# JediZ/PDE-based-image-processing

Hardware: AMD Instinct MI355X
Metric: SOR iterations/sec (3840x2160 flow) (higher is better)
Workload: dtype f32

## Files before the change

include/pdeip.h:

```cpp
#ifndef PDEIP_H
#define PDEIP_H

#ifdef __cplusplus
extern "C" {
#endif

#define PDEIP_OK 0
#define PDEIP_ERR_ARG 1
#define PDEIP_ERR_SOLVER 2
#define PDEIP_ERR_UNSUPPORTED 3
#define PDEIP_ERR_DEVICE 4
#define PDEIP_ERR_NOMEM 5

#define PDEIP_MODE_EXACT_ORDER 0
#define PDEIP_MODE_RED_BLACK 1
#define PDEIP_MODE_LINE_SCAN 2

#define PDEIP_SOLVER_SOR 1
#define PDEIP_SOLVER_ALR 2

const char *pdeip_version(void);
const char *pdeip_last_error(void);
int pdeip_set_mode(int mode);
int pdeip_get_mode(void);
int pdeip_set_device(int device_id);
int pdeip_set_devices(int n, const int *ids);
int pdeip_get_devices(int *ids, int capacity);
int pdeip_release(void);
int pdeip_last_launch_count(void);
int pdeip_debug_last_directions(int *out, int cap);
int pdeip_workspace_generation(void);
int pdeip_persist_error(void);
int pdeip_debug_raise_abort(void);
int pdeip_debug_persist_order(int B, int T, int affine, int *table);
enum { PDEIP_PLAN_ELIN4 = 0, PDEIP_PLAN_LLIN4, PDEIP_PLAN_DISP4, PDEIP_PLAN_PDE4, PDEIP_PLAN_PDE8, PDEIP_PLAN_DISPSYM4 };
enum { PDEIP_PLAN_INFO = 11, PDEIP_PLAN_RECORD = 9 };
int pdeip_debug_plan_sor(int model, int nrows, int ncols, int nframes, int iter, int mode, int aligned16, int has_dst, int num_cus,
                         int rb2_slots, int rbp_slots, int *info, int *records, int capacity);
enum { PDEIP_PLAN_ALR_ELIN4 = 0, PDEIP_PLAN_ALR_LLIN4, PDEIP_PLAN_ALR_LLIN8, PDEIP_PLAN_ALR_DISP4, PDEIP_PLAN_ALR_PDE4, PDEIP_PLAN_ALR_PDE8 };
enum { PDEIP_PLAN_ALR_INFO = 12, PDEIP_PLAN_ALR_PASS = 20 };
int pdeip_debug_plan_alr(int model, int nrows, int ncols, int nframes, int iter, int mode, int *info, int *passes);
int pdeip_debug_rcp_check(unsigned long long *counts);
int pdeip_profile_enable(int on);
int pdeip_profile_read(double *elapsed_ms, int *sweep_launches);


int pdeip_oflow_sor_elin4(const float *U, const float *V, const float *M, const float *Cu,
                          const float *Cv, const float *Du, const float *Dv, const float *wW,
                          const float *wN, const float *wE, const float *wS, int nrows, int ncols,
                          int nframes_coef, int iter, float omega, int solver, float *U_out,
                          float *V_out, float *RU, float *RV);

int pdeip_oflow_sor_llin4(const float *U, const float *V, const float *dU, const float *dV,
                          const float *M, const float *Cu, const float *Cv, const float *Du,
                          const float *Dv, const float *wW, const float *wN, const float *wE,
                          const float *wS, int nrows, int ncols, int nframes_coef, int iter,
                          float omega, int solver, float *dU_out, float *dV_out, float *RU,
                          float *RV);

int pdeip_oflow_sor_llin8(const float *U, const float *V, const float *dU, const float *dV,
                          const float *M, const float *Cu, const float *Cv, const float *Du,
                          const float *Dv, const float *wW, const float *wNW, const float *wN,
                          const float *wNE, const float *wE, const float *wSE, const float *wS,
                          const float *wSW, int nrows, int ncols, int nframes_coef, int iter,
                          float omega, int solver, float *dU_out, float *dV_out, float *RU,
                          float *RV);

int pdeip_oflow_lhs_elin4(const float *U, const float *V, const float *M, const float *Du,
                          const float *Dv, const float *wW, const float *wN, const float *wE,
                          const float *wS, int nrows, int ncols, int nframes_coef, float *AU,
                          float *AV);
// ... 421 lines not shown
```

pde-based-image-processing_amd/capi.py:

```python
import ctypes
import os

HERE = os.path.dirname(os.path.abspath(__file__))
LIB_PATH = os.environ.get("PDEIP_LIB") or os.path.join(HERE, "libpdeip.so")

PDEIP_OK = 0
PDEIP_ERR_ARG = 1
PDEIP_ERR_SOLVER = 2
PDEIP_ERR_UNSUPPORTED = 3
PDEIP_ERR_DEVICE = 4
PDEIP_ERR_NOMEM = 5
MODE_EXACT_ORDER = 0
MODE_RED_BLACK = 1
SEG_SURFACE, SEG_GREEDY, SEG_INVERSE = 0, 1, 2
MODE_LINE_SCAN = 2

_P = ctypes.c_void_p
_I = ctypes.c_int
_F = ctypes.c_float


class PdeipError(RuntimeError):

    def __init__(self, code, message):
# ... 139 lines not shown
    "pdeip_nan_resize_dev": [_P, _P, _I, _I, _I, _I, _I, ctypes.c_double, _P],
    "pdeip_inpaint_meanfill_dev": [_P, _P, _I, _I, _I, _P],
    "pdeip_tv4_inpaint_assemble_dev": [_P, _P, _P, _P, _I, ctypes.c_double, _I, _I, _I, _F] + [_P] * 6,
    "pdeip_inpaint_merge_dev": [_P, _P, _P, _I, _I, _I, _P, _P],
    "pdeip_tv_inpaint4_dev": [_P, _P, _I, _I, _I, _P, _I, _P, _P, _P],
    "pdeip_tv_inpaint4": [_P, _I, _I, _I, _P, _I, _P, _P, _P],
    "pdeip_flow_splat_dev": [_P, _P, _P, _P, _P, _I, _I, _I, ctypes.c_double, _P, _P, _P],
    "pdeip_interp_blend_dev": [_P, _P, _P, _I, _P, _P, _P, _P, _I, _I, ctypes.c_double, _P, _P],
    "pdeip_flow_interpolate_dev": [_P, _P, _P, _I, _P, _P, _P, _P, _I, _I, ctypes.c_double, _P, _P, _P, _P, _P],
    "pdeip_flow_interpolate": [_P, _P, _I, _P, _P, _P, _P, _I, _I, ctypes.c_double, _P, _P, _P, _P, _P],
    "pdeip_gauss_taps": [ctypes.c_double, _P, _I, ctypes.POINTER(ctypes.c_int)],
    "pdeip_gauss": [_P, _I, _I, _I, ctypes.c_double, _P],
    "pdeip_gauss_dev": [_P, _P, _I, _I, _I, ctypes.c_double, _P],
    "pdeip_structure_tensor_dev": [_P, _P, _I, _I, _I, ctypes.c_double, ctypes.c_double, _P],
    "pdeip_st_weights_dev": [_P, _P, _I, _I, _P, ctypes.c_double, _P, _P],
    "pdeip_st_weights_padded_dev": [_P, _P, _I, _I, _P, ctypes.c_double, _P, _P],
    "pdeip_st_pad_dev": [_P, _P, _I, _I, _I, _P, _P],
    "pdeip_st_crop_dev": [_P, _P, _I, _I, _I, _P],
    "pdeip_diffusion8": [_P, _I, _I, _I, _P, _P],
    "pdeip_diffusion8_dev": [_P, _P, _I, _I, _I, _P, _P],
    "pdeip_set_mode": [_I],
    "pdeip_get_mode": [],
    "pdeip_set_device": [_I],
    "pdeip_set_devices": [_I, ctypes.POINTER(ctypes.c_int)],
    "pdeip_get_devices": [ctypes.POINTER(ctypes.c_int), _I],
    "pdeip_release": [],
    "pdeip_last_launch_count": [],
    "pdeip_debug_last_directions": [ctypes.POINTER(ctypes.c_int), _I],
    "pdeip_workspace_generation": [],
    "pdeip_persist_error": [],
    "pdeip_debug_persist_order": [_I, _I, _I, ctypes.POINTER(ctypes.c_int)],
    "pdeip_debug_raise_abort": [],
    "pdeip_debug_plan_sor": [_I] * 11 + [ctypes.POINTER(ctypes.c_int), ctypes.POINTER(ctypes.c_int), _I],
    "pdeip_debug_plan_alr": [_I] * 6 + [ctypes.POINTER(ctypes.c_int), ctypes.POINTER(ctypes.c_int)],
    "pdeip_debug_rcp_check": [ctypes.POINTER(ctypes.c_ulonglong)],
    "pdeip_profile_enable": [_I],
    "pdeip_profile_read": [ctypes.POINTER(ctypes.c_double), ctypes.POINTER(ctypes.c_int)],
}
STRING_FUNCS = ("pdeip_version", "pdeip_last_error")

_lib = None


def load():
    global _lib
    if _lib is not None:
        return _lib
    if not os.path.exists(LIB_PATH):
        raise PdeipError(PDEIP_ERR_DEVICE,
                         "libpdeip.so is not built (%s). Run `python __graft_entry__.py build`; "
                         "there is no CPU fallback." % LIB_PATH)
    try:
        import torch
    except ImportError:
        pass
    try:
        lib = ctypes.CDLL(LIB_PATH)
    except OSError as exc:
        raise PdeipError(PDEIP_ERR_DEVICE, "cannot load %s: %s" % (LIB_PATH, exc)) from exc
    for name, argtypes in SIGNATURES.items():
        fn = getattr(lib, name)
        fn.argtypes = argtypes
        fn.restype = ctypes.c_int
    for name in STRING_FUNCS:
        fn = getattr(lib, name)
        fn.argtypes = []
# ... 58 lines not shown
```

pde-based-image-processing_amd/csrc/pdeip_sor5.hip:

```cpp
#include "pdeip_ctx.hpp"

#include "pdeip_models.hpp"
#include "pdeip_pointwise.hpp"
#include "pdeip_sor_exact.hpp"
#include "pdeip_walk_host.hpp"
#include "pdeip_persist_host.hpp"
#include "pdeip_sor_rb.hpp"
#include "pdeip_sor_rbp.hpp"
#include "pdeip_sor_small.hpp"
#include "pdeip_sor_plan.hpp"

using namespace pdeip;

namespace {

constexpr int PS = RBP_SWEEPS;

template <class Mdl> SorTraits sor_traits()
{
    using PL = RbpLayout<Mdl, PS>;
    return SorTraits{Mdl::NIT, Mdl::NCF, false, 1, RB_OWN_ROWS, PL::FITS, PL::NW, RBP_OWN_ROWS, PL::nsteps(0), &SmallLayout<Mdl>::plan, &walk_width<Mdl>};
}

template <class Mdl> auto rb_kernel(bool vec, bool first, bool two)
// ... 100 lines not shown
    RC(for_each_launch(plan, [&](const SorLaunch &l) {
        bind_buffers<Mdl>(P, buf, l);
        const bool gated = sp.nslabs > 1 && l.src == l.dst;
        if (gated) d->persist_used = true;
        hipLaunchKernelGGL(k_sor_small<Mdl>, dim3((unsigned)sp.nslabs, (unsigned)c.nframes), dim3(SL::THREADS), sp.lds, c.s, P, c.nrows, c.ncols, l.sweeps,
                           c.omega, c.col0, c.n, sp.W, gated ? counter : nullptr, abort_word);
        tls.last_launches++;
        return PDEIP_OK;
    }));
    timer.stop(plan.nlaunch);
    HIPCHK(hipGetLastError());
    return PDEIP_OK;
}

#ifndef PDEIP_TIMER_MARKERS
#define PDEIP_TIMER_MARKERS 0
#endif

template <class Mdl> int run_chain(const SweepCall<Mdl> &c, const SorPlan &plan, float *(&buf)[3][Mdl::NIT])
{
    using PL = RbpLayout<Mdl, PS>;
    SweepPlanes<Mdl> P = c.P;
    hipStream_t s = c.s;
    SweepTimer timer(s, PDEIP_TIMER_MARKERS ? 0 : plan.nlaunch);
    int done = 0;
    DeviceState *d = cur_dev();
    RC(for_each_launch(plan, [&](const SorLaunch &l) {
        bind_buffers<Mdl>(P, buf, l);
        hipEvent_t const e0 = timer.start_for(l.index), e1 = timer.stop_for(l.index);
        const int mirror = l.kind == K_RBP ? resolve_mirror(plan.mirror_mode, d->rbp_next_mirror) : 0;
        if (l.kind == K_RBP) {
            RC(ensure_lds(reinterpret_cast<const void *>(rbp_kernel<Mdl>(l.first)), PL::LDS_BYTES));
            const bool keep = l.first && done + PS < c.iter;
            launch_timed(rbp_kernel<Mdl>(l.first), dim3((unsigned)l.gridx, (unsigned)c.nframes), dim3(PL::THREADS), PL::LDS_BYTES, s, e0, e1, P, keep ? c.aux0 : nullptr,
                         keep ? c.aux1 : nullptr, c.nrows, c.ncols, l.tj, l.tiles, l.units, c.omega, c.col0, c.n, mirror);
        } else {
            launch_timed(rb_kernel<Mdl>(plan.vec, l.first, l.sweeps == 2), dim3((unsigned)l.gridx, (unsigned)c.nframes), dim3(64 * RB_WAVES_PER_BLOCK), 0, s, e0, e1, P,
                         l.first ? c.aux0 : nullptr, l.first ? c.aux1 : nullptr, c.nrows, c.ncols, l.tj, l.tiles, l.units, c.omega, c.col0, c.n);
        }
        if (l.first) {
            P.cf[Mdl::D0] = c.aux0;
            P.cf[Mdl::D1] = c.aux1;
        }
        done += l.sweeps;
        tls.last_launches++;
        tls.last_directions.push_back(mirror);
        return PDEIP_OK;
    }));
    timer.stop(plan.nlaunch);
    if (plan.copy_back)
        for (int f = 0; f < Mdl::NIT; f++) RC(copy_d2d(s, buf[BUF_CALLER][f], buf[BUF_SCRATCH][f], c.n * c.nframes));
    HIPCHK(hipGetLastError());
    return PDEIP_OK;
}

template <class Mdl>
int run_sweeps(hipStream_t s, SweepPlanes<Mdl> P, int nrows, int ncols, int nframes, int iter,
               float omega, int mode, int col0, float *const *dst = nullptr)
{
    constexpr int NIT = Mdl::NIT;
    const size_t n = (size_t)nrows * ncols;
    tls.last_launches = 0;
    tls.last_directions.clear();
    bool same = dst != nullptr, aligned = true;
    for (int f = 0; f < NIT; f++) {
        same = same && dst[f] == P.it_out[f];
        aligned = aligned && aligned16(P.it_out[f]) && (!dst || aligned16(dst[f]));
    }
// ... 23 lines not shown
}

extern "C" int pdeip_debug_plan_sor(int model, int nrows, int ncols, int nframes, int iter, int mode, int aligned16, int has_dst, int num_cus,
                                    int rb2_slots, int rbp_slots, int *info, int *records, int capacity)
{
    const char *who = "pdeip_debug_plan_sor";
    RC(check_dims(who, nrows, ncols, nframes));
    RC(check_mode(who, mode));
    if (info == nullptr || (records == nullptr && capacity > 0)) return set_err(PDEIP_ERR_ARG, "%s: null pointer", who);
    const SorShape sh{nrows, ncols, nframes, iter, mode, aligned16 != 0, has_dst != 0, 0, 0};
    const SorDevice dev{num_cus, rb2_slots, rbp_slots};
    SorPlan p;
    switch (model) {
    case PDEIP_PLAN_ELIN4: p = plan_for<ModelElin4>(sh, dev); break;
    case PDEIP_PLAN_LLIN4: p = plan_for<ModelLlin4>(sh, dev); break;
    case PDEIP_PLAN_DISP4: p = plan_for<ModelDisp4>(sh, dev); break;
    case PDEIP_PLAN_PDE4: p = plan_for<ModelPde4>(sh, dev); break;
    case PDEIP_PLAN_PDE8: p = plan_sor_pde8(sh, dev); break;
    case PDEIP_PLAN_DISPSYM4: p = plan_for<ModelDispSym4>(sh, dev); break;
    default: return set_err(PDEIP_ERR_ARG, "%s: unknown model %d", who, model);
    }
    const int head[PDEIP_PLAN_INFO] = {p.family, p.form, p.copy_back, p.copy_in, p.persist_setup, p.A, p.B, p.NC, p.W, p.last_m, 0};
    memcpy(info, head, sizeof head);
    for (int run = 0; run < (model == PDEIP_PLAN_DISPSYM4 ? 2 : 1); run++)
        (void)for_each_launch(p, [&](const SorLaunch &l) {
            const int rec[PDEIP_PLAN_RECORD] = {l.kind, l.sweeps, l.first, l.tj, l.tiles, l.units, l.gridx, l.src, l.dst};
            if (info[10] < capacity) memcpy(records + (size_t)PDEIP_PLAN_RECORD * info[10], rec, sizeof rec);
            info[10]++;
            return PDEIP_OK;
        });
    return PDEIP_OK;
}

extern "C" int pdeip_debug_persist_order(int B, int T, int affine, int *table)
{
    if (B < 1 || T < 1 || table == nullptr) return set_err(PDEIP_ERR_ARG, "pdeip_debug_persist_order: bad arguments");
    RC(use_device());
    int *dev = nullptr;
    const size_t n = PERSIST_TABLE_HDR + (size_t)B * T;
    HIPCHK(hipMalloc(&dev, n * sizeof(int)));
    hipLaunchKernelGGL(k_persist_order, dim3((unsigned)((B * T + 255) / 256)), dim3(256), 0, nullptr, dev, B, T, affine ? 1 : 0);
    const hipError_t e = hipMemcpy(table, dev, n * sizeof(int), hipMemcpyDeviceToHost);
    (void)hipFree(dev);
    if (e != hipSuccess) return set_err(PDEIP_ERR_DEVICE, "pdeip_debug_persist_order: %s", hipGetErrorString(e));
    return PDEIP_OK;
}

namespace {
__global__ void k_rcp_check(unsigned long long *counts)
{
    const unsigned long long stride = (unsigned long long)gridDim.x * blockDim.x;
    unsigned long long n = 0, bad = 0;
    for (unsigned long long i = (unsigned long long)blockIdx.x * blockDim.x + threadIdx.x; i < (1ull << 32); i += stride) {
        const unsigned bits = (unsigned)i;
        const float d = __uint_as_float(bits);
        bool in_range = true;
        RcpRange{in_range}(d);
        if (in_range != (((bits >> 23) & 0xff) >= 1 && ((bits >> 23) & 0xff) <= 252)) bad++;
        if (!in_range) continue;
        n++;
        if (__float_as_uint(RcpFast()(d)) != __float_as_uint(RcpIeee()(d))) bad++;
    }
    atomicAdd(counts + 0, n);
    atomicAdd(counts + 1, bad);
}
}
// ... 180 lines not shown
```

pde-based-image-processing_amd/csrc/pdeip_sor_plan.hpp:

```cpp
#pragma once
#include "pdeip_ctx.hpp"
#include "pdeip_sor_exact.hpp"
#include "pdeip_sor_rb.hpp"
#include "pdeip_sor_small.hpp"

namespace pdeip {

enum { SOR_NONE = 0, SOR_EXACT, SOR_SMALL, SOR_RB, SOR_RBP, SOR_PDE8 };
enum { FORM_NONE = 0, FORM_PERSIST, FORM_WALK, FORM_FRONT };
enum { K_RBP = 1, K_RB2, K_RB1, K_SMALL, K_P8C2, K_P8C1, K_PACK, K_PERSIST, K_WALK, K_DERIVE, K_FRONT, K_BORDERS };
enum { BUF_CALLER = 0, BUF_SCRATCH, BUF_DST };
constexpr int RBP_SWEEPS = 4;
constexpr int MIRROR_ALTERNATE = 3;

struct SorTraits {
    int nit, ncf;
    bool pde8;
    int ex_skew;
    int rb2_own;
    bool rbp_fits;
    int rbp_nw, rbp_own, rbp_tail;
    SmallPlan (*small)(int, int, int, int);
    int (*walk_width)(int, int, int, int);
};
struct SorShape {
    int nrows, ncols, nframes, iter, mode;
    bool aligned16, has_dst;
    size_t packed_frame_bytes;
    int persist_chunks;
};
struct SorKnobs {
    bool persist = true, walk = false, small = true, fuse = true, pipe = true;
    int small_q = 1, rb_tj = 0, rbp_tj = 0, serpentine = 0;
};
struct SorDevice { int cus, rb2_slots, rbp_slots; };
enum { FACT_CUS, FACT_RB2, FACT_RBP };

struct SorLaunch { int kind, sweeps, first, tj, tiles, units, gridx, src, dst, count, index; };
struct SorPlan {
    int family = SOR_NONE, form = FORM_NONE;
    int A = 0, B = 0, NC = 0, W = 0, last_m = 0;
    int nsteps = 0, nlaunch = 0;
    SorLaunch step[4] = {};
    bool has_dst = false, vec = false;
    int mirror_mode = 0;
    bool copy_in = false;
    bool copy_back = false;
    bool persist_setup = false;
    SmallPlan small;
    void add(int kind, int count, int sweeps = 0, int tj = 0, int tiles = 0, int units = 0, int gridx = 0)
    {
        if (count <= 0) return;
        step[nsteps++] = SorLaunch{kind, sweeps, 0, tj, tiles, units, gridx, 0, 0, count, 0};
        nlaunch += count;
    }
};

enum { KNOBS_EXACT, KNOBS_SMALL, KNOBS_CHAIN, KNOBS_PIPE };
inline void read_sor_knobs(SorKnobs &k, int set, bool pde8 = false)
{
    if (set == KNOBS_EXACT) {
        k.persist = env_int(pde8 ? "PDEIP_PDE8_PERSIST" : "PDEIP_EXACT_PERSIST", 1) != 0;
        k.walk = !pde8 && k.persist && env_int("PDEIP_EXACT_WALK", 0) != 0;
    } else if (set == KNOBS_SMALL) {
        k.small = env_int("PDEIP_RB_SMALL", 1) != 0;
        if (k.small) k.small_q = env_int("PDEIP_SMALL_Q", 1);
    } else if (set == KNOBS_CHAIN) {
        static const bool fuse_enabled = env_int("PDEIP_RB_FUSE", 1) != 0;
        k.fuse = fuse_enabled;
        k.rb_tj = g.rb_tj > 0 ? g.rb_tj : env_int("PDEIP_RB_TJ", 0);
        k.pipe = !pde8 && env_int("PDEIP_RB_PIPE", 1) != 0;
    } else {
        k.rbp_tj = env_int("PDEIP_RBP_TJ", 0);
        const char *serp = getenv("PDEIP_RBP_SERPENTINE");
        const bool set = serp && *serp;
        const int v = set ? atoi(serp) : 0;
        k.serpentine = !set ? -1 : (v < 0 || v > MIRROR_ALTERNATE ? 0 : v);
    }
}

inline bool persist_fits(int strips, int iter, size_t plane_bytes, int ncols)
{
    return strips <= 0xffff && iter <= 0x7fff && plane_bytes < 0xffff0000ull && ncols <= 65535;
}

inline int pick_rb_tj(int forced) { return forced > 0 ? (forced < 2 ? 2 : forced) : 12; }

inline int pick_rb2_tj(int slots, int tiles, int ncols, int nframes)
{
    int best = 12;
    long best_cost = -1;
    for (int tj = 2; tj <= 64; tj++) {
        const long units = (long)tiles * ((ncols + tj - 1) / tj) * nframes;
        const long cost = ((units + slots - 1) / slots) * (tj + 6);
        if (best_cost < 0 || cost <= best_cost) {
            best_cost = cost;
            best = tj;
        }
    }
    return best;
}

inline int pick_rbp_tj(int slots, int tiles, int ncols, int nframes, int tail)
{
    int best = 64;
    long best_cost = -1;
    for (int tj = 8; tj <= 1024; tj++) {
        const long units = (long)tiles * ((ncols + tj - 1) / tj) * nframes;
        const long cost = ((units + slots - 1) / slots) * (tj + tail);
        if (best_cost < 0 || cost < best_cost) {
// ... 46 lines not shown
    p.add(K_SMALL, sh.iter / per_launch, per_launch, sp.W, 1, sp.nslabs, sp.nslabs);
    p.add(K_SMALL, sh.iter % per_launch ? 1 : 0, sh.iter % per_launch, sp.W, 1, sp.nslabs, sp.nslabs);
    return true;
}

template <class Ask> inline void plan_chain(SorPlan &p, const SorTraits &t, const SorShape &sh, SorKnobs &k, const SorDevice &dev, Ask &&ask)
{
    const size_t n = (size_t)sh.nrows * sh.ncols;
    const auto strips = [&](int tj) { return (sh.ncols + tj - 1) / tj; };
    p.vec = sh.nrows % 4 == 0 && sh.aligned16;
    const bool pipe = k.pipe && k.fuse && p.vec && t.rbp_fits && (t.rbp_nw == 2 || n >= (size_t)1 << 21);
    const int n4 = pipe ? sh.iter / RBP_SWEEPS : 0, rest = sh.iter - RBP_SWEEPS * n4, n2 = k.fuse ? rest / 2 : 0, n1 = rest - 2 * n2;
    p.family = t.pde8 ? SOR_PDE8 : (n4 > 0 ? SOR_RBP : SOR_RB);
    if (n4 > 0) {
        read_sor_knobs(k, KNOBS_PIPE);
        const int tiles = (sh.nrows + t.rbp_own - 1) / t.rbp_own;
        const int tj = k.rbp_tj > 0 ? (k.rbp_tj < 2 ? 2 : k.rbp_tj)
                                    : pick_rbp_tj(dev.rbp_slots > 0 ? dev.rbp_slots : ask(FACT_RBP), tiles, sh.ncols, sh.nframes, t.rbp_tail);
        p.add(K_RBP, n4, RBP_SWEEPS, tj, tiles, tiles * strips(tj), tiles * strips(tj));
    }
    const int tj1 = pick_rb_tj(k.rb_tj), tiles1 = rb_row_tiles(sh.nrows, RB_OWN_ROWS), tiles2 = rb_row_tiles(sh.nrows, t.rb2_own);
    const int tj2 = (k.rb_tj > 0 || n2 == 0) ? tj1 : pick_rb2_tj(dev.rb2_slots > 0 ? dev.rb2_slots : ask(FACT_RB2), tiles2, sh.ncols, sh.nframes);
    const auto blocks = [](int units) { return (units + RB_WAVES_PER_BLOCK - 1) / RB_WAVES_PER_BLOCK; };
    p.add(t.pde8 ? K_P8C2 : K_RB2, n2, 2, tj2, tiles2, tiles2 * strips(tj2), blocks(tiles2 * strips(tj2)));
    p.add(t.pde8 ? K_P8C1 : K_RB1, n1, 1, tj1, tiles1, tiles1 * strips(tj1), blocks(tiles1 * strips(tj1)));
    p.copy_back = !sh.has_dst && (p.nlaunch & 1);
}

inline int default_mirror(const SorShape &sh)
{
    return (size_t)13 * sh.nrows * sh.ncols * sh.nframes * sizeof(float) > ((size_t)256 << 20) ? MIRROR_ALTERNATE : 0;
}

template <class Ask> inline SorPlan plan_sor(const SorTraits &t, const SorShape &sh, const SorDevice &dev, Ask &&ask)
{
    SorPlan p;
    SorKnobs k;
    p.has_dst = sh.has_dst;
    if (sh.iter <= 0) {
        p.copy_in = sh.has_dst;
    } else if (sh.mode != PDEIP_MODE_RED_BLACK) {
        read_sor_knobs(k, KNOBS_EXACT, t.pde8);
        plan_exact(p, t, sh, k);
    } else {
        if (!t.pde8) read_sor_knobs(k, KNOBS_SMALL);
        if (t.pde8 || !k.small || !plan_small(p, t, sh, k, dev.cus, ask)) {
            read_sor_knobs(k, KNOBS_CHAIN, t.pde8);
            plan_chain(p, t, sh, k, dev, ask);
            p.mirror_mode = k.serpentine >= 0 ? k.serpentine : default_mirror(sh);
        }
    }
    return p;
}

inline int resolve_mirror(int mode, bool &next_mirror)
{
    const int m = mode == MIRROR_ALTERNATE ? (next_mirror ? 2 : 0) : mode;
    next_mirror = m != 2;
    return m;
}

template <class F> inline int for_each_launch(const SorPlan &p, F &&fn)
{
    const int home = p.has_dst ? BUF_DST : BUF_CALLER;
    const auto out = [&](int i) -> int {
        if (p.family < SOR_RB) return home;
        if (p.has_dst) return ((p.nlaunch - 1 - i) & 1) ? BUF_SCRATCH : BUF_DST;
        return (i & 1) ? BUF_CALLER : BUF_SCRATCH;
    };
    int i = 0;
    for (int s = 0; s < p.nsteps; s++)
        for (int c = 0; c < p.step[s].count; c++, i++) {
            SorLaunch l = p.step[s];
            l.index = i;
            l.first = p.family != SOR_EXACT && i == 0;
            l.src = (i == 0 && p.family != SOR_EXACT) ? BUF_CALLER : out(i - 1);
            l.dst = out(i);
            RC(fn(l));
        }
    return PDEIP_OK;
}

// ... 4 lines not shown
```

pde-based-image-processing_amd/csrc/pdeip_sor_rbp.hpp:

```cpp
#pragma once
#include <type_traits>
#include "pdeip_sor_rb.hpp"

namespace pdeip {

constexpr int RBP_OWN_ROWS = 240;

template <class Mdl, int S> struct RbpLayout {
    static constexpr int NIT = Mdl::NIT, NRO = Mdl::NRO, NCF = Mdl::NCF;
    static constexpr int NRING = NCF + NRO;
    static constexpr int COL = 256;
    static constexpr int GROUP = NRING + NIT;
#ifndef RBP_NK_SLACK
#define RBP_NK_SLACK 1
#endif
    static constexpr int nk_for(int p) { return p + 3 * (S - 1) + RBP_NK_SLACK; }
    static constexpr int nq_for(int p) { return NRO > 0 ? p + 3 * (S - 1) + 1 : 0; }
    static constexpr size_t lds_for(int p)
    {
        return (size_t)(nk_for(p) * NCF * COL + nq_for(p) * NRO * COL + (p + 1) * NIT * COL + (S - 1) * 2 * NIT * COL) * sizeof(float);
    }
    static constexpr int pick_lead()
    {
        int best = 0;
        for (int p = 1; p <= 8; p++)
            if (lds_for(p) <= (size_t)160 * 1024 && (p - 1) * GROUP <= 63) best = p;
        return best;
    }
#ifdef RBP_LEAD
    static constexpr int P = RBP_LEAD;
#else
    static constexpr int P = pick_lead();
#endif
    static constexpr int NK = nk_for(P);
    static constexpr int NQ = nq_for(P) > 0 ? nq_for(P) : 1;
    static constexpr int NO = P + 1;
    static constexpr int K_FLOATS = NK * NCF * COL;
    static constexpr int Q_FLOATS = nq_for(P) * NRO * COL;
    static constexpr int O_FLOATS = NO * NIT * COL;
    static constexpr int H_FLOATS = (S - 1) * 2 * NIT * COL;
    static constexpr size_t LDS_BYTES = (size_t)(K_FLOATS + Q_FLOATS + O_FLOATS + H_FLOATS) * sizeof(float);
    static constexpr int NW = (NIT == 2) ? 2 : 1;
#ifndef RBP_LOADERS
#define RBP_LOADERS 1
#endif
    static constexpr int NLOAD = RBP_LOADERS;
    static constexpr int THREADS = 64 * (S * NW + NLOAD);
    static constexpr int pieces_of(int w) { return (GROUP - w + NLOAD - 1) / NLOAD; }
    static constexpr int HALO = 2 * S;
    static constexpr bool FITS = P >= 2 && LDS_BYTES <= 160 * 1024 && (P - 1) * GROUP <= 63;
    __host__ __device__ static constexpr int nsteps(int tj) { return tj + 5 * S - 1; }
};

typedef float rbp_f4 __attribute__((ext_vector_type(4)));
typedef __attribute__((address_space(3))) rbp_f4 rbp_lds_f4;
__device__ __forceinline__ void rbp_lds_read(float (&d)[4], const float *col, int lane)
{
    const rbp_f4 t = *(const rbp_lds_f4 *)(col + 4 * lane);
    d[0] = t.x; d[1] = t.y; d[2] = t.z; d[3] = t.w;
}
__device__ __forceinline__ void rbp_lds_write(float *col, int lane, const float (&d)[4])
{
    const rbp_f4 t = {d[0], d[1], d[2], d[3]};
    *(rbp_lds_f4 *)(col + 4 * lane) = t;
}

__device__ __forceinline__ void rbp_replicate_rows(float (&d)[4], bool top_lane, bool bot_lane)
{
    float a0 = d[0], a1 = d[1], a2 = d[2], a3 = d[3];
    asm("" : "+v"(a0), "+v"(a1), "+v"(a2), "+v"(a3));
    d[0] = top_lane ? a1 : a0;
    d[3] = bot_lane ? a2 : a3;
}

#ifndef RBP_AUX_COEF
#define RBP_AUX_COEF 0
#endif
#define RBP_LDS(p) ((__attribute__((address_space(3))) void *)(p))
#define RBP_GLB(p) ((const __attribute__((address_space(1))) void *)(p))

#ifdef PDEIP_RBP_STAMPS
__device__ unsigned long long g_rbp_stamps[256];
#define RBP_STAMP_T0 60
#define RBP_STAMP(n)                                                                                              \
    do {                                                                                                          \
        if (stamp_on) {                                                                                           \
            unsigned long long t_;                                                                                \
            asm volatile("s_memtime %0\n\ts_waitcnt lgkmcnt(0)" : "=s"(t_)::"memory");                            \
            if (lane == 0) g_rbp_stamps[(t - RBP_STAMP_T0) * 8 + (n)] = t_;                                        \
        }                                                                                                         \
    } while (0)
#else
#define RBP_STAMP(n)
#endif

#ifdef RBP_NO_BARRIER
__device__ __forceinline__ void rbp_barrier() { asm volatile("" ::: "memory"); }
#else
__device__ __forceinline__ void rbp_barrier() { asm volatile("s_waitcnt lgkmcnt(0)\n\ts_barrier" ::: "memory"); }
#endif
#if defined(RBP_LOADER_ONLY) && defined(RBP_SWEEPS_ONLY)
#error "RBP_LOADER_ONLY and RBP_SWEEPS_ONLY price one side each: not both"
#endif

template <class Mdl, int F0, int NF, int E0>
__device__ __forceinline__ void rbp_phase(float (&OUT)[NF][4], const float (&C)[NF][4], const float (&W)[NF][4], const float (&E)[NF][4],
                                          const float (&XC)[Mdl::NIT][4], const float (&rC)[at_least_one<Mdl::NRO>::value][4],
                                          const float (&rW)[at_least_one<Mdl::NRO>::value][4],
                                          const float (&rE)[at_least_one<Mdl::NRO>::value][4], const float (&cf)[Mdl::NCF][4],
                                          const bool (&ok)[4], float omega, float om1)
{
    constexpr int NIT = Mdl::NIT, NRO = Mdl::NRO, NRO1 = at_least_one<NRO>::value;
    float edge[NF], redge[NRO1];
#pragma unroll
    for (int f = 0; f < NF; f++) edge[f] = (E0 == 0) ? lane_above(C[f][3]) : lane_below(C[f][0]);
#pragma unroll
    for (int f = 0; f < NRO1; f++) redge[f] = (NRO == 0) ? 0.0f : ((E0 == 0) ? lane_above(rC[f][3]) : lane_below(rC[f][0]));
#pragma unroll
    for (int e = 0; e < 4; e++) {
// ... 74 lines not shown
    int koff = (((-3 * s - 1) % L::NK + L::NK) % L::NK) * KCOL, qoff = (((-3 * s) % L::NQ + L::NQ) % L::NQ) * QCOL;
    const float *const in_ring = (s == 0) ? Oring : Hring + (size_t)(s - 1) * 2 * ICOL;
    const int in_wrap = (s == 0 ? L::NO : 2) * ICOL;
    int in_off = (s == 0) ? 0 : ICOL, out_off = 0;
    float *const out_ring = Hring + (size_t)(s < S - 1 ? s : 0) * 2 * ICOL;

    auto step = [&](int t, auto mode_c, float (&Om)[NIT][4], float (&Oc)[NIT][4], float (&Op)[NIT][4], float (&Rpp)[NF][4], float (&Rp)[NF][4],
                    float (&Rc)[NF][4], const float (&Kp)[NCF][4], float (&Kc)[NCF][4], float (&Kn)[NCF][4]) __attribute__((always_inline)) {
        constexpr int MODE = decltype(mode_c)::value;
        const int x = xbase + t - 3 * s;
#ifdef PDEIP_RBP_STAMPS
        const bool stamp_on = (blockIdx.x == 100) && (s == RBP_STAMP_SWEEP) && (F0 == 0) && (t >= RBP_STAMP_T0) && (t < RBP_STAMP_T0 + 24);
#endif
        RBP_STAMP(0);
        float *const ks = Kring + koff;
        {
            const float *src = in_ring + in_off;
#pragma unroll
            for (int f = 0; f < NIT; f++) rbp_lds_read(Op[f], src + f * COL, lane);
#pragma unroll
            for (int f = 0; f < NRO1; f++)
                if (NRO > 0) {
#pragma unroll
                    for (int e = 0; e < 4; e++) {
                        Q2[f][e] = Q1[f][e];
                        Q1[f][e] = Q0[f][e];
                        Q0[f][e] = Qn[f][e];
                    }
                    rbp_lds_read(Qn[f], Qring + qoff + (NRO > 0 ? f : 0) * COL, lane);
                }
        }
        const int p = MODE < 2 ? MODE : (x + col0) & 1;
#ifdef PDEIP_RBP_STAMPS
        if (stamp_on) asm volatile("s_waitcnt lgkmcnt(0)" ::: "memory");
#endif
        RBP_STAMP(1);

        if (DERIVE) {
            constexpr int WHICH = (NF == NIT) ? 3 : (1 << F0);
            auto raw = [&](float (&k)[NCF], int e) __attribute__((always_inline)) {
#pragma unroll
                for (int f = 0; f < NCF; f++) k[f] = Kc[f][e];
                if (!Mdl::DERIVE_WE_SYMMETRIC) {
                    const float w = k[Mdl::cWW], ea = k[Mdl::cWE];
                    k[Mdl::cWW] = mirror ? ea : w;
                    k[Mdl::cWE] = mirror ? w : ea;
                }
            };
            bool in_range = true;
#pragma unroll
            for (int e = 0; e < 4; e++) {
                float k[NCF];
                raw(k, e);
                Mdl::template derive<WHICH>(k, RcpRange{in_range});
            }
            float D[2][4];
#pragma unroll
            for (int e = 0; e < 4; e++) {
                float k[NCF];
                raw(k, e);
#ifdef RBP_IEEE_DIV
                Mdl::template derive<WHICH>(k, RcpIeee());
#else
                Mdl::template derive<WHICH>(k, RcpFast());
#endif
                D[0][e] = k[Mdl::D0];
                D[1][e] = k[Mdl::D1];
// ... 91 lines not shown
                        rbp_replicate_rows(F[f], top_lane, bot_lane);
                    }
                }
            } else {
#pragma unroll
                for (int f = 0; f < NF; f++)
#pragma unroll
                    for (int e = 0; e < 4; e++) F[f][e] = Rp[f][e];
            }
        }
#undef PDEIP_RBP_PHASE
        RBP_STAMP(2);
        if (s < S - 1) {
            float *dst = out_ring + out_off;
#pragma unroll
            for (int f = 0; f < NF; f++) rbp_lds_write(dst + (F0 + f) * COL, lane, F[f]);
        } else if (store_lane && xb >= j0 && xb < j1 && (MODE < 2 || inner(xb))) {
#pragma unroll
            for (int f = 0; f < NF; f++) {
                float *out = P.it_out[F0 + f] + fo;
                rb_store4<true>(F[f], out, cmap(xb), r, nrows);
                if (MODE == 2) {
                    if (xb == 1) rb_store4<true>(F[f], out, cmap(0), r, nrows);
                    if (xb == ncols - 2) rb_store4<true>(F[f], out, cmap(ncols - 1), r, nrows);
                }
            }
        }
        koff = knext;
        if (NRO > 0) qoff = (qoff + QCOL == L::NQ * QCOL) ? 0 : qoff + QCOL;
        in_off = (in_off + ICOL == in_wrap) ? 0 : in_off + ICOL;
        out_off ^= ICOL;
        RBP_STAMP(3);
#ifdef PDEIP_RBP_STAMPS
        if (stamp_on) asm volatile("s_waitcnt lgkmcnt(0)" ::: "memory");
#endif
        RBP_STAMP(4);
        rbp_barrier();
        RBP_STAMP(5);
    };

    rbp_barrier();
#pragma unroll
    for (int f = 0; f < NCF; f++) rbp_lds_read(KB[f], Kring + koff + f * COL, lane);
    int tA = 0, tB = 0;
    {
        const int lo = 3 - xbase + 3 * s > 0 ? 3 - xbase + 3 * s : 0;
        const int hi = ncols - 3 - xbase + 3 * s < nsteps - 1 ? ncols - 3 - xbase + 3 * s : nsteps - 1;
        int ta = (lo + 2) / 3 * 3;
        if ((xbase + ta - 3 * s + col0) & 1) ta += 3;
        if (hi + 1 - ta >= 6) {
            tA = ta;
            tB = ta + (hi + 1 - ta) / 6 * 6;
        }
    }
    using M0 = std::integral_constant<int, 0>;
    using M1 = std::integral_constant<int, 1>;
    using M2 = std::integral_constant<int, 2>;
    int t = 0;
#pragma unroll 1
    for (int part = 0; part < 2; part++) {
        const int t1 = part == 0 ? tA : nsteps;
#pragma unroll 1
        for (; t < t1; t += 3) {
            step(t, M2(), O0, O1, O2, R0, R1, R2, KA, KB, KC);
            if (t + 1 < t1) step(t + 1, M2(), O1, O2, O0, R1, R2, R0, KB, KC, KA);
            if (t + 2 < t1) step(t + 2, M2(), O2, O0, O1, R2, R0, R1, KC, KA, KB);
        }
        if (part == 0) {
#pragma unroll 1
            for (; t < tB; t += 6) {
                step(t, M0(), O0, O1, O2, R0, R1, R2, KA, KB, KC);
                step(t + 1, M1(), O1, O2, O0, R1, R2, R0, KB, KC, KA);
                step(t + 2, M0(), O2, O0, O1, R2, R0, R1, KC, KA, KB);
                step(t + 3, M1(), O0, O1, O2, R0, R1, R2, KA, KB, KC);
                step(t + 4, M0(), O1, O2, O0, R1, R2, R0, KB, KC, KA);
                step(t + 5, M1(), O2, O0, O1, R2, R0, R1, KC, KA, KB);
            }
        }
    }
}

template <class Mdl, int S, bool FIRST>
__global__ void __launch_bounds__((RbpLayout<Mdl, S>::THREADS))
k_sor_rbp(SweepPlanes<Mdl> P, float *dout0, float *dout1, int nrows, int ncols, int TJ, int ntiles_r, int nunits, float omega,
          int col0, size_t frame_stride, int mirror_mode)
{
    using L = RbpLayout<Mdl, S>;
    constexpr int NIT = L::NIT, NRO = L::NRO, NCF = L::NCF, COL = L::COL, NW = L::NW;
    extern __shared__ __attribute__((aligned(16))) float rbp_lds[];
    float *const Kring = rbp_lds;
    float *const Qring = Kring + L::K_FLOATS;
    float *const Oring = Qring + L::Q_FLOATS;
    float *const Hring = Oring + L::O_FLOATS;

    const int lane = threadIdx.x & 63;
    const int wave = __builtin_amdgcn_readfirstlane(threadIdx.x >> 6);
    int unit = blockIdx.x;
    {
        const int nb = gridDim.x, per = nb >> 3;
        if (unit < (per << 3)) unit = (unit & 7) * per + (unit >> 3);
    }
    if (unit >= nunits) return;
    const size_t fo = (size_t)blockIdx.y * frame_stride;
    const int nstrips = nunits / ntiles_r;
#ifndef RBP_STRIP_MAJOR
#define RBP_STRIP_MAJOR 1
#endif
    const int a = RBP_STRIP_MAJOR ? unit % ntiles_r : unit / nstrips, b = RBP_STRIP_MAJOR ? unit / ntiles_r : unit % nstrips;
    const int r = a * RBP_OWN_ROWS - 8 + 4 * lane;
    int j0 = b * TJ, j1 = (j0 + TJ < ncols) ? j0 + TJ : ncols;
    const int mirror = mirror_mode == 2 ? 1 : (mirror_mode == 1 ? (b & 1) : 0);
    if (mirror) {
        const int t0 = ncols - j1;
        j1 = ncols - j0;
        j0 = t0;
        col0 += ncols - 1;
        const float *w = P.cf[Mdl::cWW];
        P.cf[Mdl::cWW] = P.cf[Mdl::cWE];
        P.cf[Mdl::cWE] = w;
    }
    const int nsteps = L::nsteps(TJ);
    const int xbase = j0 - L::HALO + 1 - 2;

    if (wave >= S * NW) {
        const int lw = wave - S * NW;
        const int rr = r < 0 ? 0 : (r > nrows - 4 ? nrows - 4 : r);
#ifdef RBP_SWEEPS_ONLY
        for (int t = 0; t <= nsteps; t++) rbp_barrier();
        return;
#endif
        int kslot = 0, qslot = 0, oslot = 0;
        auto issue = [&](int g) __attribute__((always_inline)) {
            const int y = xbase + 1 + g;
            const int cc = y < 0 ? 0 : (y > ncols - 1 ? ncols - 1 : y);
            const size_t off = fo + (size_t)(mirror ? ncols - 1 - cc : cc) * nrows + rr;
            float *kdst = Kring + (size_t)kslot * NCF * COL, *qdst = Qring + (size_t)qslot * NRO * COL;
#pragma unroll
            for (int f = 0; f < NCF; f++)
                if (L::NLOAD == 1 || f % L::NLOAD == lw)
                    __builtin_amdgcn_global_load_lds(RBP_GLB(P.cf[f] + off), RBP_LDS(kdst + f * COL), 16, 0, RBP_AUX_COEF);
#pragma unroll
            for (int f = 0; f < NRO; f++)
                if (L::NLOAD == 1 || (NCF + f) % L::NLOAD == lw)
                    __builtin_amdgcn_global_load_lds(RBP_GLB(P.ro[f] + off), RBP_LDS(qdst + f * COL), 16, 0, 0);
            float *odst = Oring + (size_t)oslot * NIT * COL;
#pragma unroll
            for (int f = 0; f < NIT; f++)
                if (L::NLOAD == 1 || (NCF + NRO + f) % L::NLOAD == lw)
                    __builtin_amdgcn_global_load_lds(RBP_GLB(P.it_in[f] + off), RBP_LDS(odst + f * COL), 16, 0, 0);
            kslot = (kslot + 1 == L::NK) ? 0 : kslot + 1;
            qslot = (qslot + 1 == L::NQ) ? 0 : qslot + 1;
            oslot = (oslot + 1 == L::NO) ? 0 : oslot + 1;
        };
        auto landed = [&]() __attribute__((always_inline)) {
            if (lw == 0) asm volatile("s_waitcnt vmcnt(%0)" ::"n"((L::P - 1) * L::pieces_of(0)) : "memory");
            else asm volatile("s_waitcnt vmcnt(%0)" ::"n"((L::P - 1) * L::pieces_of(L::NLOAD > 1 ? 1 : 0)) : "memory");
        };
        static_assert(L::NLOAD == 1 || L::NLOAD == 2, "one or two loader waves");
        for (int g = 0; g < L::P; g++) issue(g);
        landed();
        rbp_barrier();
#ifndef RBP_LOADER_SLEEP
#define RBP_LOADER_SLEEP 0
#endif
        for (int t = 0; t < nsteps; t++) {
#ifdef PDEIP_RBP_STAMPS
            const bool stamp_on = (blockIdx.x == 100) && (RBP_STAMP_SWEEP == 9) && (lw == 0) && (t >= RBP_STAMP_T0) && (t < RBP_STAMP_T0 + 24);
#endif
            RBP_STAMP(0);
            if (RBP_LOADER_SLEEP > 0) __builtin_amdgcn_s_sleep(RBP_LOADER_SLEEP);
            if (t + L::P <= nsteps - S) {
                issue(t + L::P);
                RBP_STAMP(1);
                landed();
            } else {
                asm volatile("s_waitcnt vmcnt(0)" ::: "memory");
            }
            RBP_STAMP(2);
            RBP_STAMP(3);
            RBP_STAMP(4);
            rbp_barrier();
            RBP_STAMP(5);
        }
        asm volatile("s_waitcnt vmcnt(0)" ::: "memory");
        return;
    }

#ifndef RBP_ROLE_REMAP
#define RBP_ROLE_REMAP 1
#endif
    const bool interior = (a * RBP_OWN_ROWS - 8 >= 1) && (a * RBP_OWN_ROWS - 8 + 255 <= nrows - 2);
#define RBP_MARCH(F0_, NF_, D_, I_)                                                                                                 \
    rbp_sweep_wave<Mdl, S, F0_, NF_, D_, I_>(P, dout0, dout1, Kring, Qring, Oring, Hring, s, lane, r, nrows, ncols, j0, j1, xbase, nsteps, omega, col0, fo, mirror)
#define RBP_ROLES(F0_, NF_)                                                                                                         \
    do {                                                                                                                            \
        if (FIRST && s == 0) {                                                                                                      \
            if (interior) RBP_MARCH(F0_, NF_, true, true);                                                                          \
            else RBP_MARCH(F0_, NF_, true, false);                                                                                  \
        } else {                                                                                                                    \
            if (interior) RBP_MARCH(F0_, NF_, false, true);                                                                         \
            else RBP_MARCH(F0_, NF_, false, false);                                                                                 \
        }                                                                                                                           \
    } while (0)
    if constexpr (NW == 2) {
        const int q = wave & 3;
        const int s = (RBP_ROLE_REMAP && S == 4) ? ((wave >> 2) << 1) | ((q == 0 || q == 3) ? 1 : 0) : wave >> 1;
        const int fld = (RBP_ROLE_REMAP && S == 4) ? (wave >> 1) & 1 : wave & 1;
        if (fld == 0) RBP_ROLES(0, 1);
        else RBP_ROLES(1, 1);
    } else {
        const int s = (RBP_ROLE_REMAP && wave < 2) ? wave ^ 1 : wave;
        RBP_ROLES(0, NIT);
    }
#undef RBP_ROLES
#undef RBP_MARCH
}

}
```

Before: 46100.

## Add optional prefetch-touch wave to RBP kernel and remap wave roles

```diff
diff --git a/include/pdeip.h b/include/pdeip.h
--- a/include/pdeip.h
+++ b/include/pdeip.h
@@ -37,6 +37,10 @@
 enum { PDEIP_PLAN_INFO = 11, PDEIP_PLAN_RECORD = 9 };
 int pdeip_debug_plan_sor(int model, int nrows, int ncols, int nframes, int iter, int mode, int aligned16, int has_dst, int num_cus,
                          int rb2_slots, int rbp_slots, int *info, int *records, int capacity);
+int pdeip_debug_plan_touch(int model, int nrows, int ncols, int nframes, int iter, int mode, int aligned16, int has_dst, int num_cus,
+                           int rb2_slots, int rbp_slots, int *touch);
+int pdeip_debug_rbp_touch(int model, int nrows, int ncols, int nframes, int tj, int mirror_mode, int touch, int unit, int frame,
+                          const unsigned *base_mis, long long *out, long long capacity, long long *count);
 enum { PDEIP_PLAN_ALR_ELIN4 = 0, PDEIP_PLAN_ALR_LLIN4, PDEIP_PLAN_ALR_LLIN8, PDEIP_PLAN_ALR_DISP4, PDEIP_PLAN_ALR_PDE4, PDEIP_PLAN_ALR_PDE8 };
 enum { PDEIP_PLAN_ALR_INFO = 12, PDEIP_PLAN_ALR_PASS = 20 };
 int pdeip_debug_plan_alr(int model, int nrows, int ncols, int nframes, int iter, int mode, int *info, int *passes);
diff --git a/pde-based-image-processing_amd/capi.py b/pde-based-image-processing_amd/capi.py
--- a/pde-based-image-processing_amd/capi.py
+++ b/pde-based-image-processing_amd/capi.py
@@ -195,6 +195,8 @@
     "pdeip_debug_persist_order": [_I, _I, _I, ctypes.POINTER(ctypes.c_int)],
     "pdeip_debug_raise_abort": [],
     "pdeip_debug_plan_sor": [_I] * 11 + [ctypes.POINTER(ctypes.c_int), ctypes.POINTER(ctypes.c_int), _I],
+    "pdeip_debug_plan_touch": [_I] * 11 + [ctypes.POINTER(ctypes.c_int)],
+    "pdeip_debug_rbp_touch": [_I] * 9 + [ctypes.POINTER(ctypes.c_uint), ctypes.POINTER(ctypes.c_longlong), ctypes.c_longlong, ctypes.POINTER(ctypes.c_longlong)],
     "pdeip_debug_plan_alr": [_I] * 6 + [ctypes.POINTER(ctypes.c_int), ctypes.POINTER(ctypes.c_int)],
     "pdeip_debug_rcp_check": [ctypes.POINTER(ctypes.c_ulonglong)],
     "pdeip_profile_enable": [_I],
diff --git a/pde-based-image-processing_amd/csrc/pdeip_sor5.hip b/pde-based-image-processing_amd/csrc/pdeip_sor5.hip
--- a/pde-based-image-processing_amd/csrc/pdeip_sor5.hip
+++ b/pde-based-image-processing_amd/csrc/pdeip_sor5.hip
@@ -156,8 +156,8 @@
         if (l.kind == K_RBP) {
             RC(ensure_lds(reinterpret_cast<const void *>(rbp_kernel<Mdl>(l.first)), PL::LDS_BYTES));
             const bool keep = l.first && done + PS < c.iter;
-            launch_timed(rbp_kernel<Mdl>(l.first), dim3((unsigned)l.gridx, (unsigned)c.nframes), dim3(PL::THREADS), PL::LDS_BYTES, s, e0, e1, P, keep ? c.aux0 : nullptr,
-                         keep ? c.aux1 : nullptr, c.nrows, c.ncols, l.tj, l.tiles, l.units, c.omega, c.col0, c.n, mirror);
+            launch_timed(rbp_kernel<Mdl>(l.first), dim3((unsigned)l.gridx, (unsigned)c.nframes), dim3(PL::THREADS - (plan.touch > 0 ? 0 : 64)), PL::LDS_BYTES, s, e0, e1, P, keep ? c.aux0 : nullptr,
+                         keep ? c.aux1 : nullptr, c.nrows, c.ncols, l.tj, l.tiles, l.units, c.omega, c.col0, c.n, mirror, plan.touch);
         } else {
             launch_timed(rb_kernel<Mdl>(plan.vec, l.first, l.sweeps == 2), dim3((unsigned)l.gridx, (unsigned)c.nframes), dim3(64 * RB_WAVES_PER_BLOCK), 0, s, e0, e1, P,
                          l.first ? c.aux0 : nullptr, l.first ? c.aux1 : nullptr, c.nrows, c.ncols, l.tj, l.tiles, l.units, c.omega, c.col0, c.n);
@@ -247,6 +247,80 @@
     return PDEIP_OK;
 }
 
+extern "C" int pdeip_debug_plan_touch(int model, int nrows, int ncols, int nframes, int iter, int mode, int aligned16, int has_dst, int num_cus,
+                                      int rb2_slots, int rbp_slots, int *touch)
+{
+    const char *who = "pdeip_debug_plan_touch";
+    RC(check_dims(who, nrows, ncols, nframes));
+    RC(check_mode(who, mode));
+    if (touch == nullptr) return set_err(PDEIP_ERR_ARG, "%s: null pointer", who);
+    const SorShape sh{nrows, ncols, nframes, iter, mode, aligned16 != 0, has_dst != 0, 0, 0};
+    const SorDevice dev{num_cus, rb2_slots, rbp_slots};
+    switch (model) {
+    case PDEIP_PLAN_ELIN4: *touch = plan_for<ModelElin4>(sh, dev).touch; break;
+    case PDEIP_PLAN_LLIN4: *touch = plan_for<ModelLlin4>(sh, dev).touch; break;
+    case PDEIP_PLAN_DISP4: *touch = plan_for<ModelDisp4>(sh, dev).touch; break;
+    case PDEIP_PLAN_PDE4: *touch = plan_for<ModelPde4>(sh, dev).touch; break;
+    case PDEIP_PLAN_PDE8: *touch = 0; break;
+    case PDEIP_PLAN_DISPSYM4: *touch = plan_for<ModelDispSym4>(sh, dev).touch; break;
+    default: return set_err(PDEIP_ERR_ARG, "%s: unknown model %d", who, model);
+    }
+    return PDEIP_OK;
+}
+
+namespace {
+template <class Mdl>
+long long touch_march(int nrows, int ncols, int tj, int mirror_mode, int touch, int unit, int frame, const unsigned *base_mis, long long *out, long long capacity)
+{
+    using PL = RbpLayout<Mdl, PS>;
+    const int tiles = (nrows + RBP_OWN_ROWS - 1) / RBP_OWN_ROWS, nunits = tiles * ((ncols + tj - 1) / tj), nsteps = PL::nsteps(tj);
+    if (unit >= nunits) return -1;
+    const RbpUnit u = rbp_unit<PS>(unit, nrows, ncols, tj, tiles, nunits, mirror_mode);
+    const size_t fo = (size_t)frame * nrows * ncols;
+    long long n = 0;
+    const auto group = [&](int t, int g) {
+        if (!PL::fetched(g, tj)) return;
+        for (int i = 0; i < rbp_touch_instructions(PL::GROUP); i++)
+            for (int lane = 0; lane < 64; lane++) {
+                int plane, k;
+                if (!rbp_touch_slot(PL::GROUP, lane, i, plane, k)) continue;
+                const long long o = rbp_touch_offset(u, g, k, base_mis[plane], nrows, ncols, fo);
+                if (o < 0) continue;
+                if (n < capacity) {
+                    const long long rec[4] = {t, g, plane, o};
+                    memcpy(out + 4 * n, rec, sizeof rec);
+                }
+                n++;
+            }
+    };
+    if (touch <= 0) return 0;
+    for (int g = PL::P; g < PL::P + touch && PL::fetched(g, tj); g++) group(-1, g);
+    for (int t = 0; t < nsteps; t++) group(t, t + PL::P + touch);
+    return n;
+}
+}
+
+extern "C" int pdeip_debug_rbp_touch(int model, int nrows, int ncols, int nframes, int tj, int mirror_mode, int touch, int unit, int frame,
+                                     const unsigned *base_mis, long long *out, long long capacity, long long *count)
+{
+    const char *who = "pdeip_debug_rbp_touch";
+    RC(check_dims(who, nrows, ncols, nframes));
+    if (base_mis == nullptr || count == nullptr || (out == nullptr && capacity > 0)) return set_err(PDEIP_ERR_ARG, "%s: null pointer", who);
+    if (nrows % 4 != 0 || tj < 2 || mirror_mode < 0 || mirror_mode > 2 || touch < 0 || touch > RBP_TOUCH_MAX || unit < 0 || frame < 0 || frame >= nframes)
+        return set_err(PDEIP_ERR_ARG, "%s: bad arguments", who);
+    long long n = -1;
+    switch (model) {
+    case PDEIP_PLAN_ELIN4: n = touch_march<ModelElin4>(nrows, ncols, tj, mirror_mode, touch, unit, frame, base_mis, out, capacity); break;
+    case PDEIP_PLAN_LLIN4: n = touch_march<ModelLlin4>(nrows, ncols, tj, mirror_mode, touch, unit, frame, base_mis, out, capacity); break;
+    case PDEIP_PLAN_DISP4: n = touch_march<ModelDisp4>(nrows, ncols, tj, mirror_mode, touch, unit, frame, base_mis, out, capacity); break;
+    case PDEIP_PLAN_PDE4: n = touch_march<ModelPde4>(nrows, ncols, tj, mirror_mode, touch, unit, frame, base_mis, out, capacity); break;
+    default: return set_err(PDEIP_ERR_ARG, "%s: model %d has no pipeline", who, model);
+    }
+    if (n < 0) return set_err(PDEIP_ERR_ARG, "%s: unit %d of a frame with fewer units", who, unit);
+    *count = n;
+    return PDEIP_OK;
+}
+
 extern "C" int pdeip_debug_persist_order(int B, int T, int affine, int *table)
 {
     if (B < 1 || T < 1 || table == nullptr) return set_err(PDEIP_ERR_ARG, "pdeip_debug_persist_order: bad arguments");
diff --git a/pde-based-image-processing_amd/csrc/pdeip_sor_plan.hpp b/pde-based-image-processing_amd/csrc/pdeip_sor_plan.hpp
--- a/pde-based-image-processing_amd/csrc/pdeip_sor_plan.hpp
+++ b/pde-based-image-processing_amd/csrc/pdeip_sor_plan.hpp
@@ -11,6 +11,7 @@
 enum { K_RBP = 1, K_RB2, K_RB1, K_SMALL, K_P8C2, K_P8C1, K_PACK, K_PERSIST, K_WALK, K_DERIVE, K_FRONT, K_BORDERS };
 enum { BUF_CALLER = 0, BUF_SCRATCH, BUF_DST };
 constexpr int RBP_SWEEPS = 4;
+constexpr int RBP_TOUCH_MAX = 1 << 16;
 constexpr int MIRROR_ALTERNATE = 3;
 
 struct SorTraits {
@@ -32,6 +33,7 @@
 struct SorKnobs {
     bool persist = true, walk = false, small = true, fuse = true, pipe = true;
     int small_q = 1, rb_tj = 0, rbp_tj = 0, serpentine = 0;
+    int touch = -1;
 };
 struct SorDevice { int cus, rb2_slots, rbp_slots; };
 enum { FACT_CUS, FACT_RB2, FACT_RBP };
@@ -44,6 +46,7 @@
     SorLaunch step[4] = {};
     bool has_dst = false, vec = false;
     int mirror_mode = 0;
+    int touch = 0;
     bool copy_in = false;
     bool copy_back = false;
     bool persist_setup = false;
@@ -76,6 +79,9 @@
         const bool set = serp && *serp;
         const int v = set ? atoi(serp) : 0;
         k.serpentine = !set ? -1 : (v < 0 || v > MIRROR_ALTERNATE ? 0 : v);
+        const char *tch = getenv("PDEIP_RBP_TOUCH");
+        const int tv = tch && *tch ? atoi(tch) : -1;
+        k.touch = tv > RBP_TOUCH_MAX ? RBP_TOUCH_MAX : tv;
     }
 }
 
@@ -188,6 +194,8 @@
     return (size_t)13 * sh.nrows * sh.ncols * sh.nframes * sizeof(float) > ((size_t)256 << 20) ? MIRROR_ALTERNATE : 0;
 }
 
+inline int default_touch(const SorShape &) { return 0; }
+
 template <class Ask> inline SorPlan plan_sor(const SorTraits &t, const SorShape &sh, const SorDevice &dev, Ask &&ask)
 {
     SorPlan p;
@@ -204,6 +212,7 @@
             read_sor_knobs(k, KNOBS_CHAIN, t.pde8);
             plan_chain(p, t, sh, k, dev, ask);
             p.mirror_mode = k.serpentine >= 0 ? k.serpentine : default_mirror(sh);
+            p.touch = p.family != SOR_RBP ? 0 : (k.touch >= 0 ? k.touch : default_touch(sh));
         }
     }
     return p;
diff --git a/pde-based-image-processing_amd/csrc/pdeip_sor_rbp.hpp b/pde-based-image-processing_amd/csrc/pdeip_sor_rbp.hpp
--- a/pde-based-image-processing_amd/csrc/pdeip_sor_rbp.hpp
+++ b/pde-based-image-processing_amd/csrc/pdeip_sor_rbp.hpp
@@ -45,12 +45,67 @@
 #define RBP_LOADERS 1
 #endif
     static constexpr int NLOAD = RBP_LOADERS;
-    static constexpr int THREADS = 64 * (S * NW + NLOAD);
+    static constexpr int THREADS = 64 * (S * NW + NLOAD + 1);
     static constexpr int pieces_of(int w) { return (GROUP - w + NLOAD - 1) / NLOAD; }
     static constexpr int HALO = 2 * S;
     static constexpr bool FITS = P >= 2 && LDS_BYTES <= 160 * 1024 && (P - 1) * GROUP <= 63;
     __host__ __device__ static constexpr int nsteps(int tj) { return tj + 5 * S - 1; }
+    __host__ __device__ static constexpr bool fetched(int g, int tj) { return g <= nsteps(tj) - S; }
 };
+
+#ifndef RBP_STRIP_MAJOR
+#define RBP_STRIP_MAJOR 1
+#endif
+struct RbpUnit {
+    int a, b;
+    int j0, j1;
+    int mirror;
+    int xbase;
+    int row0, rows;
+};
+template <int S> __host__ __device__ inline RbpUnit rbp_unit(int unit, int nrows, int ncols, int TJ, int ntiles_r, int nunits, int mirror_mode)
+{
+    RbpUnit u;
+    const int nstrips = nunits / ntiles_r;
+    u.a = RBP_STRIP_MAJOR ? unit % ntiles_r : unit / nstrips;
+    u.b = RBP_STRIP_MAJOR ? unit / ntiles_r : unit % nstrips;
+    u.j0 = u.b * TJ;
+    u.j1 = (u.j0 + TJ < ncols) ? u.j0 + TJ : ncols;
+    u.mirror = mirror_mode == 2 ? 1 : (mirror_mode == 1 ? (u.b & 1) : 0);
+    if (u.mirror) {
+        const int t0 = ncols - u.j1;
+        u.j1 = ncols - u.j0;
+        u.j0 = t0;
+    }
+    u.xbase = u.j0 - 2 * S + 1 - 2;
+    const int top = u.a * RBP_OWN_ROWS - 8, last = top + 252 > nrows - 4 ? nrows - 4 : top + 252;
+    u.row0 = top < 0 ? 0 : top;
+    u.rows = last + 4 - u.row0;
+    return u;
+}
+__host__ __device__ inline int rbp_group_column(const RbpUnit &u, int g, int ncols)
+{
+    const int y = u.xbase + 1 + g;
+    const int cc = y < 0 ? 0 : (y > ncols - 1 ? ncols - 1 : y);
+    return u.mirror ? ncols - 1 - cc : cc;
+}
+
+constexpr int RBP_TOUCH_LINES = 9;
+constexpr int rbp_touch_instructions(int planes) { return (planes * RBP_TOUCH_LINES + 63) / 64; }
+__host__ __device__ inline bool rbp_touch_slot(int planes, int lane, int i, int &plane, int &k)
+{
+    const int slot = 64 * i + lane;
+    plane = slot / RBP_TOUCH_LINES;
+    k = slot % RBP_TOUCH_LINES;
+    return plane < planes;
+}
+__host__ __device__ inline long long rbp_touch_offset(const RbpUnit &u, int g, int k, unsigned base_mis, int nrows, int ncols, size_t fo)
+{
+    const size_t off = fo + (size_t)rbp_group_column(u, g, ncols) * nrows + u.row0;
+    const unsigned mis = (base_mis + 4u * (unsigned)(off & 31)) & 127u;
+    const int delta = k == 0 ? 0 : 128 * k - (int)mis;
+    return delta < 4 * u.rows ? (long long)(off + (size_t)(delta / 4)) : -1;
+}
 
 typedef float rbp_f4 __attribute__((ext_vector_type(4)));
 typedef __attribute__((address_space(3))) rbp_f4 rbp_lds_f4;
@@ -81,10 +136,15 @@
 
 #ifdef PDEIP_RBP_STAMPS
 __device__ unsigned long long g_rbp_stamps[256];
+#ifndef RBP_STAMP_T0
 #define RBP_STAMP_T0 60
+#endif
+#ifndef RBP_STAMP_MASK
+#define RBP_STAMP_MASK 0x3f
+#endif
 #define RBP_STAMP(n)                                                                                              \
     do {                                                                                                          \
-        if (stamp_on) {                                                                                           \
+        if (stamp_on && ((RBP_STAMP_MASK >> (n)) & 1)) {                                                          \
             unsigned long long t_;                                                                                \
             asm volatile("s_memtime %0\n\ts_waitcnt lgkmcnt(0)" : "=s"(t_)::"memory");                            \
             if (lane == 0) g_rbp_stamps[(t - RBP_STAMP_T0) * 8 + (n)] = t_;                                        \
@@ -225,7 +285,7 @@
         }
         const int p = MODE < 2 ? MODE : (x + col0) & 1;
 #ifdef PDEIP_RBP_STAMPS
-        if (stamp_on) asm volatile("s_waitcnt lgkmcnt(0)" ::: "memory");
+        if (stamp_on && RBP_STAMP_MASK == 0x3f) asm volatile("s_waitcnt lgkmcnt(0)" ::: "memory");
 #endif
         RBP_STAMP(1);
 
@@ -383,7 +443,7 @@
         out_off ^= ICOL;
         RBP_STAMP(3);
 #ifdef PDEIP_RBP_STAMPS
-        if (stamp_on) asm volatile("s_waitcnt lgkmcnt(0)" ::: "memory");
+        if (stamp_on && RBP_STAMP_MASK == 0x3f) asm volatile("s_waitcnt lgkmcnt(0)" ::: "memory");
 #endif
         RBP_STAMP(4);
         rbp_barrier();
@@ -434,7 +494,7 @@
 template <class Mdl, int S, bool FIRST>
 __global__ void __launch_bounds__((RbpLayout<Mdl, S>::THREADS))
 k_sor_rbp(SweepPlanes<Mdl> P, float *dout0, float *dout1, int nrows, int ncols, int TJ, int ntiles_r, int nunits, float omega,
-          int col0, size_t frame_stride, int mirror_mode)
+          int col0, size_t frame_stride, int mirror_mode, int touch)
 {
     using L = RbpLayout<Mdl, S>;
     constexpr int NIT = L::NIT, NRO = L::NRO, NCF = L::NCF, COL = L::COL, NW = L::NW;
@@ -453,26 +513,61 @@
     }
     if (unit >= nunits) return;
     const size_t fo = (size_t)blockIdx.y * frame_stride;
-    const int nstrips = nunits / ntiles_r;
-#ifndef RBP_STRIP_MAJOR
-#define RBP_STRIP_MAJOR 1
-#endif
-    const int a = RBP_STRIP_MAJOR ? unit % ntiles_r : unit / nstrips, b = RBP_STRIP_MAJOR ? unit / ntiles_r : unit % nstrips;
+    const RbpUnit u = rbp_unit<S>(unit, nrows, ncols, TJ, ntiles_r, nunits, mirror_mode);
+    const int a = u.a, j0 = u.j0, j1 = u.j1, mirror = u.mirror;
     const int r = a * RBP_OWN_ROWS - 8 + 4 * lane;
-    int j0 = b * TJ, j1 = (j0 + TJ < ncols) ? j0 + TJ : ncols;
-    const int mirror = mirror_mode == 2 ? 1 : (mirror_mode == 1 ? (b & 1) : 0);
     if (mirror) {
-        const int t0 = ncols - j1;
-        j1 = ncols - j0;
-        j0 = t0;
         col0 += ncols - 1;
         const float *w = P.cf[Mdl::cWW];
         P.cf[Mdl::cWW] = P.cf[Mdl::cWE];
         P.cf[Mdl::cWE] = w;
     }
     const int nsteps = L::nsteps(TJ);
-    const int xbase = j0 - L::HALO + 1 - 2;
-
+    const int xbase = u.xbase;
+
+    if (wave == S * NW + L::NLOAD) {
+        if (touch <= 0) return;
+#ifdef RBP_SWEEPS_ONLY
+        for (int t = 0; t <= nsteps; t++) rbp_barrier();
+        return;
+#endif
+        constexpr int NI = rbp_touch_instructions(L::GROUP);
+        const float *base[NI];
+        unsigned mis[NI];
+        int kk[NI];
+        bool on[NI];
+#pragma unroll
+        for (int i = 0; i < NI; i++) {
+            int pl;
+            on[i] = rbp_touch_slot(L::GROUP, lane, i, pl, kk[i]);
+            const float *p = P.cf[0];
+#pragma unroll
+            for (int f = 1; f < NCF; f++) p = (pl == f) ? P.cf[f] : p;
+#pragma unroll
+            for (int f = 0; f < NRO; f++) p = (pl == NCF + f) ? P.ro[f] : p;
+#pragma unroll
+            for (int f = 0; f < NIT; f++) p = (pl == NCF + NRO + f) ? P.it_in[f] : p;
+            base[i] = p;
+            mis[i] = (unsigned)(size_t)p & 127u;
+        }
+        unsigned sink = 0;
+        auto touch_group = [&](int g) __attribute__((always_inline)) {
+            if (!L::fetched(g, TJ)) return;
+#pragma unroll
+            for (int i = 0; i < NI; i++) {
+                const long long o = rbp_touch_offset(u, g, kk[i], mis[i], nrows, ncols, fo);
+                if (on[i] && o >= 0) asm volatile("global_load_dword %0, %1, off" : "+v"(sink) : "v"(base[i] + o));
+            }
+        };
+        for (int g = L::P; g < L::P + touch && L::fetched(g, TJ); g++) touch_group(g);
+        rbp_barrier();
+        for (int t = 0; t < nsteps; t++) {
+            touch_group(t + L::P + touch);
+            rbp_barrier();
+        }
+        asm volatile("s_waitcnt vmcnt(0)" : "+v"(sink));
+        return;
+    }
     if (wave >= S * NW) {
         const int lw = wave - S * NW;
         const int rr = r < 0 ? 0 : (r > nrows - 4 ? nrows - 4 : r);
@@ -482,9 +577,7 @@
 #endif
         int kslot = 0, qslot = 0, oslot = 0;
         auto issue = [&](int g) __attribute__((always_inline)) {
-            const int y = xbase + 1 + g;
-            const int cc = y < 0 ? 0 : (y > ncols - 1 ? ncols - 1 : y);
-            const size_t off = fo + (size_t)(mirror ? ncols - 1 - cc : cc) * nrows + rr;
+            const size_t off = fo + (size_t)rbp_group_column(u, g, ncols) * nrows + rr;
             float *kdst = Kring + (size_t)kslot * NCF * COL, *qdst = Qring + (size_t)qslot * NRO * COL;
 #pragma unroll
             for (int f = 0; f < NCF; f++)
@@ -520,7 +613,7 @@
 #endif
             RBP_STAMP(0);
             if (RBP_LOADER_SLEEP > 0) __builtin_amdgcn_s_sleep(RBP_LOADER_SLEEP);
-            if (t + L::P <= nsteps - S) {
+            if (L::fetched(t + L::P, TJ)) {
                 issue(t + L::P);
                 RBP_STAMP(1);
                 landed();
@@ -555,12 +648,12 @@
     } while (0)
     if constexpr (NW == 2) {
         const int q = wave & 3;
-        const int s = (RBP_ROLE_REMAP && S == 4) ? ((wave >> 2) << 1) | ((q == 0 || q == 3) ? 1 : 0) : wave >> 1;
-        const int fld = (RBP_ROLE_REMAP && S == 4) ? (wave >> 1) & 1 : wave & 1;
+        const int s = (RBP_ROLE_REMAP && S == 4) ? ((wave >> 2) << 1) | (q < 2 ? 1 : 0) : wave >> 1;
+        const int fld = wave & 1;
         if (fld == 0) RBP_ROLES(0, 1);
         else RBP_ROLES(1, 1);
     } else {
-        const int s = (RBP_ROLE_REMAP && wave < 2) ? wave ^ 1 : wave;
+        const int s = (RBP_ROLE_REMAP && S >= 3 && wave < 3) ? (wave + 1) % 3 : wave;
         RBP_ROLES(0, NIT);
     }
 #undef RBP_ROLES
```

After: 45930, median of 2. Within noise of the previous version (-0.4%).
